# Guivernoir/ICS-WT-PhysicsEngine

Hardware: AMD Instinct MI355X
Metric: reactor-zone-steps/sec (higher is better)
Workload: dtype f64

## Files before the change

ics-wt-physicsengine_amd/csrc/wt_numjac.hpp:

```cpp
#pragma once
#include <hip/hip_runtime.h>
#include <stdint.h>
#include "wt_tables.hpp"
#include "wt_lanes.hpp"
#include "wt_rhs.hpp"
#include "wt_pcr.hpp"

namespace wt {

struct FdCols { double D[3][3]; double S[3][3]; };

struct ZoneProps { double H, iw, phi, kT, rho; bool bpos; };

struct FdBase { double k_lo, k_hi, kd, H_lo, H_hi, C_lo, C_hi, T_lo, T_hi, rho_hi; };

template <bool ROW>
__device__ __forceinline__ FdBase fd_base(const Lane &L, const RK &k, const double y[3], const ZoneProps &b)
{
    FdBase n;
    n.rho_hi = from_hi<ROW, 1>(L, b.rho);
    n.k_hi = k_above(k, b.rho, n.rho_hi);
    n.k_lo = keep_m(L.m_lo[0], from_lo<ROW, 1>(L, n.k_hi));
    n.kd = k_diag(k, n.k_lo, n.k_hi);
    n.H_lo = keep_m(L.m_lo[0], from_lo<ROW, 1>(L, b.H)); n.H_hi = keep_m(L.m_hi[0], from_hi<ROW, 1>(L, b.H));
    n.C_lo = keep_m(L.m_lo[0], from_lo<ROW, 1>(L, y[SCL])); n.C_hi = keep_m(L.m_hi[0], from_hi<ROW, 1>(L, y[SCL]));
    n.T_lo = keep_m(L.m_lo[0], from_lo<ROW, 1>(L, y[STT])); n.T_hi = keep_m(L.m_hi[0], from_hi<ROW, 1>(L, y[STT]));
    return n;
}

template <bool ROW, int SP, class KC>
__device__ __forceinline__ void fd_species_pass(const Lane &L, const KC &kc, const RK &k, const double y[3], const double f[3],
                                                const ZoneProps &b, const FdBase &n, double hcol, bool colmask, bool all_cols,
                                                FdCols &out, bool &bad, double &badval)
{
    const double ypert = y[SP] + hcol;
#pragma unroll
    for (int q = 0; q < 3; ++q)
#pragma unroll
        for (int r = 0; r < 3; ++r) { out.D[q][r] = 0.0; out.S[q][r] = 0.0; }
    auto put = [&](int q, int r, double fn) { out.D[q][r] = fn - f[q]; out.S[q][r] = fmax(fabs(f[q]), fabs(fn)); };
    const double kphi = b.kT * b.phi;
    if constexpr (SP == SPH) {
        PropPH p = prop_pH(kc, k, ypert);
        if (!all_cols && !colmask) { p.H = b.H; p.iw = b.iw; p.phi = b.phi; }
        const double Hx_lo = keep_m(L.m_lo[0], from_lo<ROW, 1>(L, p.H)), Hx_hi = keep_m(L.m_hi[0], from_hi<ROW, 1>(L, p.H));
        put(SPH, 1, row_pH(k, mix3(n.k_lo, n.k_hi, n.kd, n.H_lo, n.H_hi, p.H), p.H, p.iw));
        put(SCL, 1, row_Cl(k, mix3(n.k_lo, n.k_hi, n.kd, n.C_lo, n.C_hi, y[SCL]), y[SCL], b.kT * p.phi));
        put(SPH, 0, row_pH(k, mix3(n.k_lo, n.k_hi, n.kd, Hx_lo, n.H_hi, b.H), b.H, b.iw));
        put(SPH, 2, row_pH(k, mix3(n.k_lo, n.k_hi, n.kd, n.H_lo, Hx_hi, b.H), b.H, b.iw));
    }
    if constexpr (SP == SCL) {
        const double cx = (all_cols || colmask) ? ypert : y[SCL];
        const double Cx_lo = keep_m(L.m_lo[0], from_lo<ROW, 1>(L, cx)), Cx_hi = keep_m(L.m_hi[0], from_hi<ROW, 1>(L, cx));
        put(SCL, 1, row_Cl(k, mix3(n.k_lo, n.k_hi, n.kd, n.C_lo, n.C_hi, cx), cx, kphi));
        put(SCL, 0, row_Cl(k, mix3(n.k_lo, n.k_hi, n.kd, Cx_lo, n.C_hi, y[SCL]), y[SCL], kphi));
        put(SCL, 2, row_Cl(k, mix3(n.k_lo, n.k_hi, n.kd, n.C_lo, Cx_hi, y[SCL]), y[SCL], kphi));
    }
    if constexpr (SP == STT) {
        PropT p = prop_T(kc, ypert);
        if (colmask && p.bad && !bad) { bad = true; badval = ypert; }
        double tx = ypert;
        if (!all_cols && !colmask) { p.kT = b.kT; p.rho = b.rho; tx = y[STT]; }
        const double Tx_lo = keep_m(L.m_lo[0], from_lo<ROW, 1>(L, tx)), Tx_hi = keep_m(L.m_hi[0], from_hi<ROW, 1>(L, tx));
        const double khi_own = k_above(k, p.rho, n.rho_hi);
        const double khi_up = k_above(k, b.rho, from_hi<ROW, 1>(L, p.rho));
        const double klo_own = keep_m(L.m_lo[0], from_lo<ROW, 1>(L, khi_up));
        const double klo_dn = keep_m(L.m_lo[0], from_lo<ROW, 1>(L, khi_own));
        {
            const double kd = k_diag(k, klo_own, khi_own);
            put(SPH, 1, row_pH(k, mix3(klo_own, khi_own, kd, n.H_lo, n.H_hi, b.H), b.H, b.iw));
            put(SCL, 1, row_Cl(k, mix3(klo_own, khi_own, kd, n.C_lo, n.C_hi, y[SCL]), y[SCL], p.kT * b.phi));
            put(STT, 1, row_T(k, mix3(klo_own, khi_own, kd, n.T_lo, n.T_hi, tx), tx));
        }
        {
            const double kd = k_diag(k, klo_dn, n.k_hi);
            put(SPH, 0, row_pH(k, mix3(klo_dn, n.k_hi, kd, n.H_lo, n.H_hi, b.H), b.H, b.iw));
            put(SCL, 0, row_Cl(k, mix3(klo_dn, n.k_hi, kd, n.C_lo, n.C_hi, y[SCL]), y[SCL], kphi));
            put(STT, 0, row_T(k, mix3(klo_dn, n.k_hi, kd, Tx_lo, n.T_hi, y[STT]), y[STT]));
        }
        {
            const double kd = k_diag(k, n.k_lo, khi_up);
            put(SPH, 2, row_pH(k, mix3(n.k_lo, khi_up, kd, n.H_lo, n.H_hi, b.H), b.H, b.iw));
            put(SCL, 2, row_Cl(k, mix3(n.k_lo, khi_up, kd, n.C_lo, n.C_hi, y[SCL]), y[SCL], kphi));
            put(STT, 2, row_T(k, mix3(n.k_lo, khi_up, kd, n.T_lo, Tx_hi, y[STT]), y[STT]));
        }
    }
}

template <bool ROW, int SP>
__device__ __forceinline__ void fd_col_reduce(const Lane &L, const FdCols &c, double &maxd, double &scale)
{
    maxd = -1.0; scale = 0.0;
#pragma unroll
    for (int q = 0; q < 3; ++q) {
        const bool dep_nb = (q == SP) || (SP == STT);
        const bool dep_own = dep_nb || (q == SCL && SP == SPH);
        if (!dep_own) continue;
        double d_lo = 0, s_lo = 0, d_hi = 0, s_hi = 0;
        if (dep_nb) {
            d_lo = from_lo<ROW, 1>(L, c.D[q][2]); s_lo = from_lo<ROW, 1>(L, c.S[q][2]);
            d_hi = from_hi<ROW, 1>(L, c.D[q][0]); s_hi = from_hi<ROW, 1>(L, c.S[q][0]);
        }
        if (dep_nb && L.has_lo && fabs(d_lo) > maxd) { maxd = fabs(d_lo); scale = s_lo; }
        if (fabs(c.D[q][1]) > maxd) { maxd = fabs(c.D[q][1]); scale = c.S[q][1]; }
        if (dep_nb && L.has_hi && fabs(d_hi) > maxd) { maxd = fabs(d_hi); scale = s_hi; }
    }
}

__device__ __forceinline__ double fd_step(double y, double fac, double ysc)
{
    return __dadd_rn(__dadd_rn(y, __dmul_rn(fac, ysc)), -y);
}

template <bool ROW, int SP, class KC>
__device__ __forceinline__ void num_jac_species(const Lane &L, const KC &kc, const RK &k, const double y[3], const double f[3],
                                                const ZoneProps &b, const FdBase &nb, double &fac, FdCols &cols, bool &bad, double &badval)
{
    const double fs = (f[SP] >= 0) ? 1.0 : -1.0;
    const double ysc = fs * fmax(ATOL, fabs(y[SP]));
    double h = fd_step(y[SP], fac, ysc);
    while (WT_RARE(h == 0)) { fac *= 10; h = fd_step(y[SP], fac, ysc); }
    fd_species_pass<ROW, SP>(L, kc, k, y, f, b, nb, h, true, true, cols, bad, badval);
    double maxd, scl;
    fd_col_reduce<ROW, SP>(L, cols, maxd, scl);
    const bool small = maxd < rc::NJ_REJECT * scl;
    if (WT_RARE(__ballot(small) != 0ull)) {
        const double nf = 10 * fac;
        const double hn = fd_step(y[SP], nf, ysc);
        FdCols c2;
        fd_species_pass<ROW, SP>(L, kc, k, y, f, b, nb, hn, small, false, c2, bad, badval);
        double md2, sc2;
        fd_col_reduce<ROW, SP>(L, c2, md2, sc2);
        const bool upd = small && (maxd * sc2 < md2 * scl);
        if (upd) { fac = nf; h = hn; maxd = md2; scl = sc2; }
        const int iu = upd ? 1 : 0;
        const int iu_lo = __shfl_up(iu, 1, 64), iu_hi = __shfl_down(iu, 1, 64);
        const bool upd_lo = L.has_lo && (iu_lo != 0), upd_hi = L.has_hi && (iu_hi != 0);
#pragma unroll
        for (int q = 0; q < 3; ++q) {
            if (upd_lo) cols.D[q][0] = c2.D[q][0];
            if (upd) cols.D[q][1] = c2.D[q][1];
            if (upd_hi) cols.D[q][2] = c2.D[q][2];
        }
    }
    const double h_lo = from_lo<ROW, 1>(L, h), h_hi = from_hi<ROW, 1>(L, h);
    const double ih0 = L.has_lo ? rcp(h_lo) : 0.0, ih1 = rcp(h), ih2 = L.has_hi ? rcp(h_hi) : 0.0;
#pragma unroll
    for (int q = 0; q < 3; ++q) { cols.D[q][0] *= ih0; cols.D[q][1] *= ih1; cols.D[q][2] *= ih2; }
    const bool sm = maxd < rc::NJ_SMALL * scl, bg = maxd > rc::NJ_BIG * scl;
    if (sm) fac *= 10;
    if (bg) fac *= 0.1;
    fac = fmax(fac, rc::NJ_MINF);
}

template <bool ROW, class KTP>
__device__ __forceinline__ void num_jac(const Lane &L, const RKStore &ks, KTP ktab, const double y[3], const double f[3],
                                        double fac[3], bool &have_fac, Jac &J, bool &bad, double &badval, bool &t_dense)
{
    if (!have_fac) { fac[0] = fac[1] = fac[2] = rc::NJ_F0; have_fac = true; }
    FdCols cols;
    ZoneProps b;
    FdBase nb;
    {
        const KT ct = load_kt(ktab());
        const PropT bpt = prop_T(ct, y[STT]);
        b.kT = bpt.kT; b.rho = bpt.rho;
    }
    {
        const KP cp = load_kp(ktab());
        const RK k = fetch_reactor(ks);
        const PropPH bpp = prop_pH(cp, k, y[SPH]);
        b.H = bpp.H; b.iw = bpp.iw; b.phi = bpp.phi; b.bpos = bpp.bpos;
        nb = fd_base<ROW>(L, k, y, b);
        num_jac_species<ROW, SPH>(L, cp, k, y, f, b, nb, fac[SPH], cols, bad, badval);
#pragma unroll
        for (int r = 0; r < 3; ++r) J.pp[r] = cols.D[SPH][r];
        J.cp = cols.D[SCL][1];
    }
    {
        const RK k = fetch_reactor(ks);
        num_jac_species<ROW, SCL>(L, 0, k, y, f, b, nb, fac[SCL], cols, bad, badval);
#pragma unroll
        for (int r = 0; r < 3; ++r) J.cc[r] = cols.D[SCL][r];
    }
    {
        const KT ct = load_kt(ktab());
        const RK k = fetch_reactor(ks);
        num_jac_species<ROW, STT>(L, ct, k, y, f, b, nb, fac[STT], cols, bad, badval);
#pragma unroll
        for (int r = 0; r < 3; ++r) { J.tt[r] = cols.D[STT][r]; J.pt[r] = cols.D[SPH][r]; J.ct[r] = cols.D[SCL][r]; }
        t_dense = jac_t_dense(J) || (ct.dense_bias != 0.0);
    }
}

}
```

ics-wt-physicsengine_amd/csrc/wt_step.hpp:

```cpp
#pragma once
#include <hip/hip_runtime.h>
#include <stdint.h>
#include "wt_tables.hpp"
#include "wt_args.hpp"
#include "wt_lanes.hpp"
#include "wt_rhs.hpp"
#include "wt_pcr.hpp"
#include "wt_numjac.hpp"
#include "wt_queue.hpp"

namespace wt {

template <bool ROW, int LV = 6>
__device__ __forceinline__ double rms3(const Lane &L, const double x[3], const double sc[3])
{
    double s = 0.0;
#pragma unroll
    for (int q = 0; q < 3; ++q) { const double v = x[q] * rcp(sc[q]); s += v * v; }
    return sqrt_k(div_by(seg_sum<ROW, LV>(L, s), L.d3n));
}

__device__ __forceinline__ double ulp_above(double t)
{
    return __longlong_as_double(__double_as_longlong(t) + 1) - t;
}

__device__ __forceinline__ double predict_factor(double h_abs, bool have_old, double h_abs_old,
                                                 double error_norm, double error_norm_old)
{
    double mult = 1.0;
    const double ie = rcp(error_norm);
    if (have_old && error_norm != 0) mult = h_abs * rcp(h_abs_old) * root4(error_norm_old * ie);
    return fmin(1.0, mult) * root4(ie);
}

struct Flag {
    uint32_t &w; const uint32_t m;
    __device__ __forceinline__ operator bool() const { return (w & m) != 0u; }
    __device__ __forceinline__ Flag &operator=(bool v) { w = v ? (w | m) : (w & ~m); return *this; }
    __device__ __forceinline__ Flag &operator=(const Flag &o) { return *this = (bool)o; }
    __device__ __forceinline__ Flag &operator|=(bool v) { w = v ? (w | m) : w; return *this; }
};

enum Phase : int {
    PH_OUTER_BEGIN = 0,
    PH_INIT_STEP,
    PH_F1,
    PH_STEP_BEGIN,
    PH_ATTEMPT,
    PH_NEWTON,
    PH_ERR_REFINE,
    PH_FNEW,
    PH_DONE
};

struct SolverCounters { int nfev, njev, nlu, nsteps, nrej; };

template <int LV> struct LdsMap {
    static constexpr int RK_DOUBLES = RK_UNI * rk_maxr(LV) + rk_lane_doubles(LV);
    static constexpr int HIST_DOUBLES = rk_maxr(LV);
    static constexpr int F_DOUBLES = FSlots<LV>::LDS_SLOTS * 64;
    static constexpr int IO_DOUBLES = (int)((sizeof(wts::StepIO) + 7) / 8);
    static constexpr int TAIL_DOUBLES = F_DOUBLES > IO_DOUBLES ? F_DOUBLES : IO_DOUBLES;
    static constexpr int X_OFF = RK_DOUBLES + HIST_DOUBLES, X_DOUBLES = 64;
    static constexpr int F_OFF = (X_OFF + X_DOUBLES + 1) & ~1;
    static constexpr int TOTAL = F_OFF + TAIL_DOUBLES;
    static_assert(X_OFF >= (LV >= 2 ? (1 << (LV - 2)) : 0), "reads below the exchange row must stay inside the allocation");
};

template <bool ROW, int NS>
__device__ __forceinline__ void rhs_points(const Lane &L, const RKStore &ks, ArgPtr pa, const double (*y)[3], double (*F)[3], bool *bad)
{
    PropPH pp[NS]; PropT pt[NS];
    {
        ArgPtr a = fresh(pa);
        const KP c = load_kp(&a->kt);
        const RK k = fetch_reactor(ks);
        double x[NS];
#pragma unroll
        for (int s = 0; s < NS; ++s) x[s] = y[s][SPH];
        prop_pH_n<NS>(c, k, x, pp);
    }
    __builtin_amdgcn_sched_barrier(0);
    {
        ArgPtr a = fresh(pa);
        const KT c = load_kt(&a->kt);
        double x[NS];
#pragma unroll
        for (int s = 0; s < NS; ++s) x[s] = y[s][STT];
        prop_T_n<NS>(c, x, pt);
#pragma unroll
        for (int s = 0; s < NS; ++s) bad[s] = pt[s].bad;
    }
    {
        const RK k = fetch_reactor(ks);
#pragma unroll
        for (int s = 0; s < NS; ++s)
            rhs_rows<ROW>(L, k, pp[s].H, pp[s].iw, pp[s].bpos, pt[s].kT * pp[s].phi, pt[s].rho, y[s][SCL], y[s][STT], F[s]);
    }
}

__host__ __device__ constexpr bool first_attempt_in_probe_trip(int , bool ) { return true; }

template <int LV, bool ROW>
__device__ __forceinline__ void run_item(ArgPtr pa, const Lane &L, double *lds, int group, int step0, int cnt)
{
    using M = LdsMap<LV>;
    ArgPtr a = fresh(pa);
    const int n_zones = L.n, R = a->R;
    const int lane = threadIdx.x & 63, seg = lane / n_zones;
    const int64_t q_first = (int64_t)group * R;
    const int64_t q_end = a->q_ctrl ? a->N : a->r1;
    const bool present = (seg < R) && (q_first + seg < q_end);
    const int64_t r = present ? (int64_t)a->perm[q_first + seg] : 0;
    const int64_t idx = r * n_zones + L.z;
    const double dt = a->dt;
    const int step_limit = a->step_limit, sens_on = a->sens.on, plc_on = a->sens.plc_on;
    const bool want_diag = a->wave_diag != nullptr;
    const RKStore ks = {lds + seg, lds + RK_UNI * rk_maxr(LV) + lane, rk_maxr(LV), L.m_lo[0], L.m_hi[0], rk_lane_in_lds(LV)};
    int *hist0 = reinterpret_cast<int *>(lds + M::RK_DOUBLES);
    int *rix = hist0 + rk_maxr(LV);
    double *lds_factors = lds + M::F_OFF;
    wts::StepIO &io = *reinterpret_cast<wts::StepIO *>(lds_factors);

    double y0[3] = {7.0, 1.0, 20.0};
    double f[3] = {0, 0, 0};
    double t_out = 0;
    double dH = 0, dR = 0, dK = 0, badval = 0;
    double flow_used = 0;
    uint32_t st = 0;
    bool frozen = !present, f_valid = false, wrote_k = false, raised = false;
    int steps_done = 0, reads_done = 0, cost_acc = 0;
    SolverCounters last_cnt = {0, 0, 0, 0, 0};
    int diag_trips = 0, diag_newton = 0;
#ifdef WT_STAMPS
    int diag_fact = 0, diag_jac = 0, diag_f3 = 0;
#define WT_COUNT(c) ++(c)
#else
    constexpr int diag_fact = 0, diag_jac = 0, diag_f3 = 0;
#define WT_COUNT(c) do { } while (0)
#endif
#ifdef WT_STAMPS
    long long sec[8] = {0, 0, 0, 0, 0, 0, 0, 0}; long long tprev = __builtin_amdgcn_s_memtime();
#define WT_STAMP(i) do { const long long tn_ = __builtin_amdgcn_s_memtime(); sec[i] += tn_ - tprev; tprev = tn_; } while (0)
#else
#define WT_STAMP(i) do { } while (0)
#endif
    const long long clk0 = want_diag ? __builtin_amdgcn_s_memtime() : 0, wall0 = want_diag ? __builtin_amdgcn_s_memrealtime() : 0;
    if (present) {
        st = a->status[r];
        if (st & (ST_T_RANGE | ST_T_RANGE_POST)) frozen = true;
        y0[SPH] = a->pH[idx]; y0[SCL] = a->Cl[idx]; y0[STT] = a->T[idx];
        t_out = a->time[r];
        const double *bc = a->sched ? a->sched + (int64_t)(a->first_step + step0) * NB * a->N : a->bc;
        RK k0; load_reactor(a->par, bc, a->N, r, n_zones, k0); mask_reactor_for_lane(L, k0);
        park_reactor(ks, k0);
        if (sens_on && L.z == 0) hist0[seg] = a->sens.hist_value ? a->sens.hist_pos[r] : 0;
        if (L.z == 0) rix[seg] = (int)r;
    }

    for (int k = 0; k < cnt; ++k) {
        bool stepped = false;
        if (!frozen) {
          if (WT_RARE(seg_any(L, !(isfinite(y0[0]) && isfinite(y0[1]) && isfinite(y0[2]))))) { st |= ST_NONFINITE; frozen = true; }
          else {
            double yc[3], W[3][3];
            double aux[3] = {0, 0, 0};
            constexpr bool HELD = LV <= 5;
            typedef Held<HELD> AReg64;
            AReg64 Qa[3][3], y_old_a[3], sol_t_old_a, sol_h_a;
#pragma unroll
            for (int q = 0; q < 3; ++q) { y_old_a[q].init(); Qa[q][0].init(); Qa[q][1].init(); Qa[q][2].init(); }
            sol_t_old_a.init(); sol_h_a.init();
            Jac J;
            JacA<(LV <= 4)> ja; ja.init();
            FStore<LV> F;
            F.cell = (LdsDouble2 *)lds_factors + lane;
            uint32_t fl = 1u << 4;
            Flag have_fac{fl, 1u << 0}, have_old{fl, 1u << 1}, have_old_l{fl, 1u << 2}, have_sol{fl, 1u << 3}, current_jac{fl, 1u << 4},
                 have_lu{fl, 1u << 5}, rejected{fl, 1u << 6}, keep_h{fl, 1u << 7}, have_norm_old{fl, 1u << 8}, have_rate{fl, 1u << 9},
                 bad{fl, 1u << 10}, failed{fl, 1u << 11}, fv{fl, 1u << 12}, need_jac{fl, 1u << 13},
                 limit_hit{fl, 1u << 16}, pend_f{fl, 1u << 17}, jac_after_fnew{fl, 1u << 18},
                 j_dense{fl, 1u << 19};
            fv = f_valid;
            AReg64 fac_a[3]; fac_a[0].init(); fac_a[1].init(); fac_a[2].init();
            double t = t_out, t_bound = t_out + dt, max_step = fmin(dt, 10.0);
            double h = 0, t_new = 0, h_abs = 0, h_abs_l = 0, min_step = 0;
            AReg64 h_abs_old_a, err_old_a, h_abs_old_l_a, err_old_l_a;
            h_abs_old_a.init(); err_old_a.init(); h_abs_old_l_a.init(); err_old_l_a.init();
            int kk = 0, n_iter = 0; double dW_norm_old = 0, rate = 0;
            double error_norm = 0, safety = 0;
            double d0 = 0, d1 = 0, h0 = 0;
            SolverCounters cnt_s = {0, 0, 0, 0, 0};
            int attempts = 0;
            int badstage = 0;
            int phase = PH_OUTER_BEGIN;
#pragma unroll
            for (int q = 0; q < 3; ++q) { yc[q] = y0[q]; W[0][q] = W[1][q] = W[2][q] = 0.0; }

            auto initial_step_first_half = [&]() {
                double sc[3];
#pragma unroll
                for (int q = 0; q < 3; ++q) sc[q] = ATOL + fabs(yc[q]) * RTOL;
                d0 = rms3<ROW, LV>(L, yc, sc); d1 = rms3<ROW, LV>(L, f, sc);
                h0 = (d0 < 1e-5 || d1 < 1e-5) ? 1e-6 : 0.01 * d0 * rcp(d1);
                h0 = fmin(h0, fabs(t_bound - t));
#pragma unroll
                for (int q = 0; q < 3; ++q) aux[q] = yc[q] + h0 * f[q];
            };
            auto reject_step = [&]() {
                const double fct = predict_factor(h_abs_l, have_old_l, h_abs_old_l_a.get(), error_norm, err_old_l_a.get());
                h_abs_l *= fmax(MIN_FACTOR, safety * fct);
                have_lu = false; rejected = true; cnt_s.nrej++;
                phase = PH_ATTEMPT;
            };
            auto accept_step = [&]() {
                const bool recompute_jac = (n_iter > 2) && have_rate && (rate > 1e-3);
                double fct = predict_factor(h_abs_l, have_old_l, h_abs_old_l_a.get(), error_norm, err_old_l_a.get());
                fct = fmin(MAX_FACTOR, safety * fct);
                if (!recompute_jac && fct < 1.2) fct = 1.0; else have_lu = false;
                h_abs_old_a.set(h_abs);
                err_old_a.set(error_norm);
                have_old = true;
                h_abs = h_abs_l * fct;
                const KZ kz = lit_kz(); const KA ka = lit_ka();
#pragma unroll
                for (int q = 0; q < 3; ++q) {
                    const ZRow z = z_of_w(kz, W, q);
                    y_old_a[q].set(yc[q]);
                    Qa[q][0].set(z.z0 * ka.P[0] + z.z1 * ka.P[3] + z.z2 * ka.P[6]);
                    Qa[q][1].set(z.z0 * ka.P[1] + z.z1 * ka.P[4] + z.z2 * ka.P[7]);
                    Qa[q][2].set(z.z0 * ka.P[2] + z.z1 * ka.P[5] + z.z2 * ka.P[8]);
                    yc[q] = yc[q] + z.z2;
                }
                sol_t_old_a.set(t); sol_h_a.set(t_new - t); have_sol = true;
                t = t_new;
                cnt_s.nsteps++; cnt_s.nfev++;
                pend_f = true; fv = false;
                current_jac = recompute_jac;
                const bool more = (t - t_bound) < 0;
                if (recompute_jac || !more) { jac_after_fnew = recompute_jac; phase = PH_FNEW; }
                else phase = PH_STEP_BEGIN;
            };

            if (fv) {
                cnt_s.nfev++;
                phase = PH_INIT_STEP;
            }

            WT_STAMP(0);
            while (true) {
                if (__ballot(phase != PH_DONE) == 0ull) break;
                if (phase == PH_INIT_STEP) {
                    initial_step_first_half();
                    phase = PH_F1;
                }
                if (phase == PH_STEP_BEGIN) {
                    min_step = 10 * fabs(ulp_above(t));
                    if (h_abs > max_step) { h_abs_l = max_step; have_old_l = false; }
                    else if (h_abs < min_step) { h_abs_l = min_step; have_old_l = false; }
                    else { h_abs_l = h_abs; have_old_l = have_old; h_abs_old_l_a.set(h_abs_old_a.get()); err_old_l_a.set(err_old_a.get()); }
                    rejected = false; keep_h = false;
                    phase = PH_ATTEMPT;
                }
                if (phase == PH_ATTEMPT) {
                    if (!keep_h) {
                        if (WT_RARE(step_limit > 0 && attempts >= step_limit)) { failed = true; limit_hit = true; phase = PH_DONE; }
                        else if (WT_RARE(h_abs_l < min_step)) { failed = true; phase = PH_DONE; }
                        else {
                            attempts++;
                            h = h_abs_l;
                            t_new = t + h;
                            if (t_new - t_bound > 0) t_new = t_bound;
                            h = t_new - t;
                            h_abs_l = fabs(h);
                        }
                    }
                    if (phase == PH_ATTEMPT) {
                        keep_h = false;
                        double Z0[3][3];
                        if (!have_sol) {
#pragma unroll
                            for (int s = 0; s < 3; ++s)
#pragma unroll
                                for (int q = 0; q < 3; ++q) Z0[s][q] = 0.0;
                        } else {
                            const double sol_t_old = sol_t_old_a.get(), isol = rcp(sol_h_a.get());
                            double Q[3][3], y_old[3];
#pragma unroll
                            for (int q = 0; q < 3; ++q) { y_old[q] = y_old_a[q].get(); Q[q][0] = Qa[q][0].get(); Q[q][1] = Qa[q][1].get(); Q[q][2] = Qa[q][2].get(); }
                            const KG kg = load_kg(&fresh(pa)->rt);
                            const double cs[3] = {kg.C0, kg.C1, 1.0};
#pragma unroll
                            for (int s = 0; s < 3; ++s) {
                                const double x = ((t + h * cs[s]) - sol_t_old) * isol;
                                const double p1 = x * x, p2 = p1 * x;
#pragma unroll
                                for (int q = 0; q < 3; ++q)
                                    Z0[s][q] = (__builtin_fma(Q[q][2], p2, __builtin_fma(Q[q][0], x, Q[q][1] * p1)) + y_old[q]) - yc[q];
                            }
                        }
                        const KN kn0 = load_kn(&fresh(pa)->rt);
#pragma unroll
                        for (int q = 0; q < 3; ++q) {
                            W[0][q] = kn0.TI[0] * Z0[0][q] + kn0.TI[1] * Z0[1][q] + kn0.TI[2] * Z0[2][q];
                            W[1][q] = kn0.TI[3] * Z0[0][q] + kn0.TI[4] * Z0[1][q] + kn0.TI[5] * Z0[2][q];
                            W[2][q] = kn0.TI[6] * Z0[0][q] + kn0.TI[7] * Z0[1][q] + kn0.TI[8] * Z0[2][q];
                        }
                        kk = 0; have_norm_old = false; have_rate = false; rate = 0.0;
                        phase = PH_NEWTON;
                    }
                }
                WT_STAMP(1);
                const bool newton = (phase == PH_NEWTON);
                diag_trips++;
                const bool eval0 = (phase == PH_OUTER_BEGIN || phase == PH_F1 || phase == PH_ERR_REFINE || phase == PH_FNEW || newton);
                const bool eval3 = newton && pend_f;
                double ye[3][3], Fe[3][3];
#pragma unroll
                for (int q = 0; q < 3; ++q) {
                    double p0 = yc[q];
                    if (phase == PH_F1) p0 = aux[q];
                    if (phase == PH_ERR_REFINE) p0 = yc[q] + aux[q];
                    ye[0][q] = p0;
                }
                auto stage_points = [&]() {
                    const KZ kzp = load_kz(&fresh(pa)->rt);
#pragma unroll
                    for (int q = 0; q < 3; ++q) {
                        const ZRow z = z_of_w(kzp, W, q);
                        if (newton) ye[0][q] = yc[q] + z.z0;
                        ye[1][q] = yc[q] + z.z1; ye[2][q] = yc[q] + z.z2;
                    }
                };
                if constexpr (LV >= 5) stage_points();
                bool b0 = false, b1 = false, b2 = false, b3 = false;
                if (__ballot(newton) != 0ull) {
                    if constexpr (LV < 5) stage_points();
                    bool bb[3];
                    rhs_points<ROW, 3>(L, ks, pa, ye, Fe, bb);
                    b0 = bb[0] && eval0; b1 = bb[1] && newton; b2 = bb[2] && newton;
                    if (eval0 && phase != PH_FNEW) cnt_s.nfev++;
                    if (newton) cnt_s.nfev += 2;
                } else if (__ballot(eval0) != 0ull) {
                    bool bb[1];
                    rhs_points<ROW, 1>(L, ks, pa, ye, Fe, bb);
                    b0 = bb[0] && eval0;
                    if (eval0 && phase != PH_FNEW) cnt_s.nfev++;
                }
                if (__ballot(eval3) != 0ull) {
                    WT_COUNT(diag_f3);
                    double fy[1][3]; bool bb[1];
                    rhs_points<ROW, 1>(L, ks, pa, &yc, fy, bb);
                    b3 = bb[0] && eval3;
                    if (eval3) {
                        pend_f = false;
#pragma unroll
                        for (int q = 0; q < 3; ++q) f[q] = fy[0][q];
                    }
                }
                if (WT_RARE(__ballot(b0 || b1 || b2 || b3) != 0ull)) {
                    const bool mine = b0 || b1 || b2 || b3;
                    if (mine && !bad) {
                        badstage = b3 ? 0 : (b0 ? 1 : (b1 ? 2 : 3));
                        badval = b3 ? yc[STT] : (b0 ? ye[0][STT] : (b1 ? ye[1][STT] : ye[2][STT]));
                    }
                    bad |= mine;
                    if (seg_any(L, bad)) { raised = true; phase = PH_DONE; }
                }

                if (WT_RARE(phase == PH_OUTER_BEGIN)) {
#pragma unroll
                    for (int q = 0; q < 3; ++q) f[q] = Fe[0][q];
                    phase = PH_INIT_STEP;
                } else if (phase == PH_F1) {
                    double sc[3], df[3];
#pragma unroll
                    for (int q = 0; q < 3; ++q) { sc[q] = ATOL + fabs(yc[q]) * RTOL; df[q] = Fe[0][q] - f[q]; }
                    const double d2 = rms3<ROW, LV>(L, df, sc) * rcp(h0);
                    double h1;
                    if (d1 <= 1e-15 && d2 <= 1e-15) h1 = fmax(1e-6, h0 * 1e-3);
                    else h1 = root4(0.01 * rcp(fmax(d1, d2)));
                    h_abs = fmin(fmin(100 * h0, h1), fmin(fabs(t_bound - t), max_step));
                    need_jac = true;
                    if constexpr (!first_attempt_in_probe_trip(LV, ROW)) phase = PH_STEP_BEGIN;
                    else {
                        min_step = 10 * fabs(ulp_above(t));
                        h_abs_l = (h_abs < min_step) ? min_step : h_abs;
                        attempts++;
                        h = h_abs_l;
                        t_new = t + h;
                        if (t_new - t_bound > 0) t_new = t_bound;
                        h = t_new - t;
                        h_abs_l = fabs(h);
#pragma unroll
                        for (int s = 0; s < 3; ++s)
#pragma unroll
                            for (int q = 0; q < 3; ++q) Fe[s][q] = f[q];
                        cnt_s.nfev += 3;
                        phase = PH_NEWTON;
                    }
                } else if (phase == PH_FNEW) {
#pragma unroll
                    for (int q = 0; q < 3; ++q) f[q] = Fe[0][q];
                    pend_f = false;
                    fv = true;
                    if (jac_after_fnew) { need_jac = true; jac_after_fnew = false; }
                    phase = ((t - t_bound) < 0) ? PH_STEP_BEGIN : PH_DONE;
                }

                WT_STAMP(3);
#ifdef WT_STAMPS
                if (__ballot(need_jac) != 0ull) WT_COUNT(diag_jac);
#endif
                if (need_jac) {
                    bool jbad = false, hf = have_fac, jd = false; double jval = 0;
                    asm volatile("" ::: "memory");
                    double fac[3] = {fac_a[0].get(), fac_a[1].get(), fac_a[2].get()};
                    num_jac<ROW>(L, ks, [&]() { return &fresh(pa)->kt; }, yc, f, fac, hf, J, jbad, jval, jd); cnt_s.njev++;
                    fac_a[0].set(fac[0]); fac_a[1].set(fac[1]); fac_a[2].set(fac[2]);
                    have_fac = hf;
                    j_dense = jd;
                    ja.put(J);
                    need_jac = false;
                    if (WT_RARE(seg_any(L, jbad))) {
                        if (jbad) { badstage = 0; badval = jval; }
                        bad |= jbad; raised = true; phase = PH_DONE;
                    }
                }
                WT_STAMP(5);
#ifdef WT_STAMPS
                if (__ballot(phase == PH_NEWTON && !have_lu) != 0ull) WT_COUNT(diag_fact);
#endif
                if (phase == PH_NEWTON && !have_lu) {
                    { Jac Jb; ja.bands(Jb); factorize<ROW, LV>(L, Jb, h, F); } have_lu = true; cnt_s.nlu += 2;
                }

                WT_STAMP(2);
                if (__ballot(phase == PH_NEWTON) != 0ull) diag_newton++;
                if (phase == PH_NEWTON) {
                    Jac Jc; ja.coupling(Jc);
                    bool finite = true;
#pragma unroll
                    for (int s = 0; s < 3; ++s)
#pragma unroll
                        for (int q = 0; q < 3; ++q) finite = finite && isfinite(Fe[s][q]);
                    bool conv = false, diverged = false;
                    if (WT_RARE(!seg_all(L, finite))) {
                        diverged = true;
                    } else {
                        const double ih = rcp(h);
                        const RTabPtr rt = &fresh(pa)->rt;
                        const KN kn = load_kn(rt); const KZ kz = load_kz(rt);
                        const double M_real = kn.mu_r * ih, Mcr = kn.mu_cr * ih, Mci = kn.mu_ci * ih;
                        double fr[3], fcr[3], fci[3], scale[3];
#pragma unroll
                        for (int q = 0; q < 3; ++q) {
                            scale[q] = kz.atol + fabs(yc[q]) * kz.rtol;
                            fr[q] = (Fe[0][q] * kn.TI[0] + Fe[1][q] * kn.TI[1] + Fe[2][q] * kn.TI[2]) - M_real * W[0][q];
                            const double re = Fe[0][q] * kn.TI[3] + Fe[1][q] * kn.TI[4] + Fe[2][q] * kn.TI[5];
                            const double im = Fe[0][q] * kn.TI[6] + Fe[1][q] * kn.TI[7] + Fe[2][q] * kn.TI[8];
                            fcr[q] = re - (Mcr * W[1][q] - Mci * W[2][q]);
                            fci[q] = im - (Mcr * W[2][q] + Mci * W[1][q]);
                        }
                        solve_rc<ROW, LV>(L, Jc, F, fr, fcr, fci, __ballot(j_dense) == 0ull);
                        double ssum = 0.0;
#pragma unroll
                        for (int q = 0; q < 3; ++q) {
                            const double is = rcp(scale[q]);
                            const double u = fr[q] * is, v = fcr[q] * is, w = fci[q] * is;
                            ssum += u * u + v * v + w * w;
                        }
                        const double dW_norm = sqrt_k(div_by(seg_sum<ROW, LV>(L, ssum), L.d9n));
                        if (have_norm_old) { rate = dW_norm * rcp(dW_norm_old); have_rate = true; }
                        const double i1r = rcp(1 - rate);
                        if (have_rate && (rate >= 1 || powi6(rate, NEWTON_MAXITER - kk) * i1r * dW_norm > kn.newton_tol)) {
                            diverged = true;
                        } else {
#pragma unroll
                            for (int q = 0; q < 3; ++q) { W[0][q] += fr[q]; W[1][q] += fcr[q]; W[2][q] += fci[q]; }
                            if (dW_norm == 0 || (have_rate && rate * i1r * dW_norm < kn.newton_tol)) conv = true;
                            dW_norm_old = dW_norm; have_norm_old = true;
                        }
                    }
                    n_iter = kk + 1;
                    kk++;
                    if (!conv && !diverged && kk == NEWTON_MAXITER) diverged = true;
                    if (WT_RARE(diverged)) {
                        if (current_jac) { h_abs_l *= 0.5; have_lu = false; cnt_s.nrej++; phase = PH_ATTEMPT; }
                        else { need_jac = true; current_jac = true; have_lu = false; keep_h = true; phase = PH_ATTEMPT; }
                    } else if (conv) {
                        double err[3], esc[3];
                        const double ih_e = rcp(h);
                        const KZ kze = lit_kz(); const KE ke = lit_ke();
#pragma unroll
                        for (int q = 0; q < 3; ++q) {
                            const ZRow z = z_of_w(kze, W, q);
                            const double ZE = (z.z0 * ke.E0 + z.z1 * ke.E1 + z.z2 * ke.E2) * ih_e;
                            err[q] = f[q] + ZE;
                            esc[q] = kze.atol + fmax(fabs(yc[q]), fabs(yc[q] + z.z2)) * kze.rtol;
                        }
                        solve_real<ROW, LV>(L, Jc, F, err, __ballot(j_dense) == 0ull);
                        error_norm = rms3<ROW, LV>(L, err, esc);
                        safety = 0.9 * (2 * NEWTON_MAXITER + 1) / (2 * NEWTON_MAXITER + n_iter);
                        if (WT_RARE(rejected && error_norm > 1)) {
#pragma unroll
                            for (int q = 0; q < 3; ++q) aux[q] = err[q];
                            phase = PH_ERR_REFINE;
                        } else if (WT_RARE(error_norm > 1)) {
                            reject_step();
                        } else {
                            accept_step();
                        }
                    }
                } else if (WT_RARE(phase == PH_ERR_REFINE)) {
                    Jac Jc; ja.coupling(Jc);
                    double err[3], esc[3];
                    const double ih_e = rcp(h);
                    const KZ kze = lit_kz(); const KE ke = lit_ke();
#pragma unroll
                    for (int q = 0; q < 3; ++q) {
                        const ZRow z = z_of_w(kze, W, q);
                        const double ZE = (z.z0 * ke.E0 + z.z1 * ke.E1 + z.z2 * ke.E2) * ih_e;
                        err[q] = Fe[0][q] + ZE;
                        esc[q] = kze.atol + fmax(fabs(yc[q]), fabs(yc[q] + z.z2)) * kze.rtol;
                    }
                    solve_real<ROW, LV>(L, Jc, F, err, __ballot(j_dense) == 0ull);
                    error_norm = rms3<ROW, LV>(L, err, esc);
                    if (error_norm > 1) reject_step(); else accept_step();
                }
                WT_STAMP(4);
            }
            last_cnt = cnt_s;
            cost_acc += cnt_s.nfev;

            if (WT_RARE(raised)) {
                st |= ST_T_RANGE; frozen = true;
                double v = badval; int best = 1 << 30;
#pragma unroll 1
                for (int sidx = 0; sidx < 5; ++sidx) {
                    const unsigned long long m = __ballot(bad && badstage == sidx) & L.segmask;
                    if (m != 0ull && best == (1 << 30)) { best = sidx; v = __shfl(badval, (int)__builtin_ctzll(m), 64); }
                }
                badval = v;
                raised = false;
            } else {
                if (failed) st |= ST_SOLVER_FAILED;
                if (limit_hit) st |= ST_STEP_LIMIT;
#pragma unroll
                for (int q = 0; q < 3; ++q) y0[q] = yc[q];
                stepped = true; steps_done++;
                t_out = t_out + dt;
                flow_used = ks.uni[15 * ks.stride];
                double dHv; PropT pt;
                {
                    ArgPtr a2 = fresh(pa);
                    const KP cp = load_kp(&a2->kt); const KT ct = load_kt(&a2->kt);
                    dHv = exp10_k(cp, -y0[SPH]); pt = prop_T(ct, y0[STT]);
                }
                dH = dHv;
                dR = pt.rho;
                bool clamped = false;
                if (WT_RARE(seg_any(L, pt.bad))) {
                    st |= ST_T_RANGE_POST; frozen = true;
                    const unsigned long long m = __ballot(pt.bad) & L.segmask;
                    badval = __shfl(y0[STT], (int)__builtin_ctzll(m), 64);
                } else {
                    dK = pt.kT; wrote_k = true;
                    if (WT_RARE(seg_any(L, y0[SPH] < 0 || y0[SPH] > 14))) { st |= ST_CLAMP_PH; y0[SPH] = fmin(fmax(y0[SPH], 0.0), 14.0); clamped = true; }
                    if (WT_RARE(seg_any(L, y0[SCL] < 0))) { st |= ST_CLAMP_CL; y0[SCL] = fmax(y0[SCL], 0.0); clamped = true; }
                    if (WT_RARE(seg_any(L, y0[STT] < 0 || y0[STT] > 100))) { st |= ST_CLAMP_T; y0[STT] = fmin(fmax(y0[STT], 0.0), 100.0); clamped = true; }
                    f_valid = fv && !clamped && !failed;
                }
            }
          }
        }

        WT_STAMP(6);
        if constexpr (prog_in_item(LV)) {
          if (WT_RARE(fresh(pa)->scr.on)) {
            ArgPtr s = fresh(pa);
            static_assert(M::TAIL_DOUBLES >= wtsc::STAGE_DOUBLES, "the score program stages the zones' state in the factor store");
            const bool live = present && stepped && !(st & ST_T_RANGE_POST);
            wtsc::evaluate(s->scr, live, L.z, n_zones, lane, L.base, r, t_out, y0, lds_factors,
                           s->scr.step0 + s->first_step + step0 + k);
          }
        }
        if constexpr (prog_in_item(LV)) {
          const int dst_on = fresh(pa)->dst.on, trn_on = fresh(pa)->trn.on;
          if (WT_RARE((dst_on | trn_on) != 0)) {
            ArgPtr d = fresh(pa);
            const bool live = present && stepped && !(st & ST_T_RANGE_POST);
            bool reload = false;
            double q0 = 0.0;
            if (trn_on && d->trn.jct.on && present && !L.has_hi) q0 = d->bc[r];
            if (dst_on) {
                if (live && L.z == 0) wtd::evaluate(d->dst, r, t_out, d->bc, d->N, ExpK());
                reload = live;
            }
            static_assert(M::TAIL_DOUBLES >= wtr::PARK_Q * wtr::PARK_SEGS, "a junction program parks the outlets in the factor store");
            if (trn_on) reload = wtr::feed(d->trn, present, live, !L.has_hi, seg, n_zones, r, t_out, y0, q0, d->bc, d->N, lds_factors, JctK()) || reload;
            __syncthreads();
            if (reload) {
                RK k1; load_reactor(d->par, d->bc, d->N, r, n_zones, k1); mask_reactor_for_lane(L, k1);
                park_reactor(ks, k1);
                f_valid = false;
            }
          }
        }
        if (sens_on) {
            ArgPtr b = fresh(pa);
            __syncthreads();
            if (seg < R) {
                const bool live = stepped && !(st & ST_T_RANGE_POST);
                if (L.z == 0) {
                    io.stepped[seg] = live ? 1 : 0;
                    if (live) reads_done++;
                    io.t_after[seg] = t_out;
                    io.tap[0][seg] = (float)y0[SPH]; io.tap[2][seg] = (float)y0[SCL]; io.tap[4][seg] = (float)y0[STT];
                    io.tap[6][seg] = (float)flow_used;
                }
                if (!L.has_hi) { io.tap[1][seg] = (float)y0[SPH]; io.tap[3][seg] = (float)y0[SCL]; io.tap[5][seg] = (float)y0[STT]; }
            }
            __syncthreads();
            if constexpr (prog_in_item(LV)) wts::suite_step(b->sens, b->ins, io, rix, R, hist0, k, wtsv::Program());
            else wts::suite_step(b->sens, b->ins, io, rix, R, hist0, k);
            if (plc_on) {
                const int gs = b->first_step + step0 + k;
                const bool scan = ((gs + 1) % b->sens.scan_every == 0) || (gs + 1 == b->call_steps);
                __syncthreads();
                if constexpr (prog_in_item(LV)) {
                  if (scan && WT_RARE(fresh(pa)->wir.on)) {
                    ArgPtr wp = fresh(pa);
                    wtw::route(wp->wir, wp->trn.length, lane < R && io.stepped[lane], lane, rix, io);
                  }
                }
                if (lane < R && io.stepped[lane]) {
                    const int64_t rr = rix[lane];
                    const double lt = b->sens.pack.loop_time[rr];
                    if (scan) {
                        const bool inj = prog_in_item(LV) && WT_RARE(fresh(pa)->inj.on);
                        if (inj) wti::tamper_sensors(fresh(pa)->inj, rr, &io.val[0][lane], &io.fault[0][lane], wts::RMAX, lt + dt);
                        wtp::pack_inputs(b->sens.pack, rr, &io.val[0][lane], &io.fault[0][lane], wts::RMAX, lt);
                        double c[3];
                        const bool act = prog_in_item(LV) && WT_RARE(fresh(pa)->act.on);
                        const double row0 = act ? b->sens.cmd.bc[rr] : 0.0;
                        double inlet_v;
                        if (inj) inlet_v = wtp::apply_commands(b->sens.cmd, rr, c, wti::command_tamper(fresh(pa)->inj, rr, lt + dt));
                        else inlet_v = wtp::apply_commands(b->sens.cmd, rr, c);
                        if (prog_in_item(LV) && WT_RARE(fresh(pa)->alm.on)) wta::override_commands(fresh(pa)->alm, b->sens.cmd, rr, c);
                        if (act) wtv::actuate(fresh(pa)->act, b->sens.cmd, rr, c, inlet_v, row0, lt + dt);
                        io.cmd[0][lane] = c[0]; io.cmd[1][lane] = c[1]; io.cmd[2][lane] = c[2];
                    }
                    b->sens.pack.loop_time[rr] = lt + dt;
                }
                int owned = 0;
                if constexpr (prog_in_item(LV)) {
                  if (scan && WT_RARE(fresh(pa)->tun.on) && lane < R && io.stepped[lane]) {
                    ArgPtr up = fresh(pa);
                    const int64_t rr = rix[lane];
                    owned = wtu::tune_execute(up->tun, up->ctl, rr, &io.val[0][lane], &io.fault[0][lane], wts::RMAX, up->sens.pack.loop_time[rr]);
                  }
                }
                if (scan && WT_RARE(fresh(pa)->ctl.on) && lane < R && io.stepped[lane]) {
                    ArgPtr cp = fresh(pa);
                    const int64_t rr = rix[lane];
                    wtc::pi_execute(cp->ctl, rr, &io.val[0][lane], &io.fault[0][lane], wts::RMAX, cp->sens.pack.loop_time[rr], owned);
                }
                if (prog_in_item(LV) && scan && WT_RARE(fresh(pa)->alm.on) && lane < R && io.stepped[lane]) {
                    ArgPtr ap = fresh(pa);
                    const int64_t rr = rix[lane];
                    wta::evaluate(ap->alm, rr, ap->sens.N, &io.val[0][lane], &io.fault[0][lane], wts::RMAX, ap->sens.out_value,
                                  ap->sens.out_fault, ap->sens.pack.loop_time[rr]);
                }
                if constexpr (prog_in_item(LV)) {
                  if (scan && WT_RARE(fresh(pa)->det.on) && lane < R && io.stepped[lane]) {
                    ArgPtr dp = fresh(pa);
                    const int64_t rr = rix[lane];
                    wtk::evaluate(dp->det, rr, dp->sens.N, &io.val[0][lane], &io.fault[0][lane], wts::RMAX, dp->sens.out_value,
                                  dp->sens.out_fault, dp->sens.pack.loop_time[rr]);
                  }
                }
                if constexpr (prog_in_item(LV)) {
                  if (scan && WT_RARE(fresh(pa)->trd.on) && lane < R && io.stepped[lane]) {
                    ArgPtr tp = fresh(pa);
                    const int64_t rr = rix[lane];
                    wtt::record(*tp, rr, &io.val[0][lane], &io.fault[0][lane], &io.cmd[0][lane], wts::RMAX, tp->sens.pack.loop_time[rr]);
                  }
                }
                if (scan) {
                    __syncthreads();
                    if (present && io.stepped[seg]) {
                        RK k0; load_reactor(b->par, b->bc, b->N, r, n_zones, k0, &io.cmd[0][seg], wts::RMAX); mask_reactor_for_lane(L, k0);
                        park_reactor(ks, k0);
                        f_valid = false;
                    }
                }
            }
            __syncthreads();
        }
        if constexpr (x_in_item(LV)) {
          if (WT_RARE(fresh(pa)->x_on)) {
            ArgPtr x = fresh(pa);
            const int gs = x->first_step + step0 + k;
            if (x->rec_pH) {
                const unsigned m = (unsigned)x->rec_phase + (unsigned)gs + 1u, every = (unsigned)x->rec_every;
                const unsigned slot = (unsigned)x->rec_slot0 + m / every - 1u;
                if (m % every == 0u && slot < (unsigned)x->rec_cap && present) {
                    const int64_t row = (int64_t)slot * x->N;
                    const int64_t o = row * n_zones + idx;
                    x->rec_pH[o] = y0[SPH]; x->rec_Cl[o] = y0[SCL]; x->rec_T[o] = y0[STT];
                    if (L.z == 0) {
                        x->rec_time[row + r] = t_out;
                        x->rec_flow[row + r] = steps_done > 0 ? flow_used : x->flow[r];
                        x->rec_status[row + r] = st;
                    }
                }
            }
            if (x->sched && k + 1 < cnt) {
                if (present) {
                    RK k1; load_reactor(x->par, x->sched + (int64_t)(gs + 1) * NB * x->N, x->N, r, n_zones, k1);
                    mask_reactor_for_lane(L, k1);
                    park_reactor(ks, k1);
                }
                f_valid = false;
            }
          }
        }
        WT_STAMP(7);
    }

    ArgPtr c = fresh(pa);
    if (present) {
        if (steps_done > 0) {
            c->pH[idx] = y0[SPH]; c->Cl[idx] = y0[SCL]; c->T[idx] = y0[STT];
            c->dH[idx] = dH; c->dRho[idx] = dR;
            if (wrote_k) c->dK[idx] = dK;
        }
        if (L.z == 0) {
            if (steps_done > 0) {
                c->time[r] = t_out;
                c->flow[r] = flow_used;
                if (c->stats) {
                    int32_t *o = c->stats + r * 5;
                    o[0] = last_cnt.nfev; o[1] = last_cnt.njev; o[2] = last_cnt.nlu; o[3] = last_cnt.nsteps; o[4] = last_cnt.nrej;
                }
                if (sens_on && c->sens.hist_value) c->sens.hist_pos[r] = hist0[seg] + reads_done;
            }
            c->status[r] = st;
            if (st & (ST_T_RANGE | ST_T_RANGE_POST)) c->bad_T[r] = badval;
            if (c->cost && cost_acc > 0) c->cost[r] += cost_acc;
        }
    }
    if (want_diag && lane == 0) {
        unsigned long long *o = reinterpret_cast<unsigned long long *>(c->wave_diag + (int64_t)group * WT_DIAG_SLOTS);
        atomicAdd(o + 0, (unsigned long long)diag_trips); atomicAdd(o + 1, (unsigned long long)diag_newton);
        atomicAdd(o + 2, (unsigned long long)(__builtin_amdgcn_s_memtime() - clk0));
        atomicAdd(o + 3, (unsigned long long)(__builtin_amdgcn_s_memrealtime() - wall0));
        atomicAdd(o + 4, (unsigned long long)diag_fact); atomicAdd(o + 5, (unsigned long long)diag_jac);
        atomicAdd(o + 6, (unsigned long long)diag_f3); atomicAdd(o + 7, 1ull);
#ifdef WT_STAMPS
        for (int i = 0; i < 8; ++i) atomicAdd(o + 8 + i, (unsigned long long)sec[i]);
#endif
    }
}

}
```

Before: 1.726 billion.

## Restructure Radau step loop to skip redundant RHS and property evaluations

Several schedule changes go into the implicit solver loop. The outer-begin RHS evaluation is hoisted ahead of the first trip, and its base properties are handed to the numerical Jacobian so they are not recomputed. The pending f evaluation is folded into the Newton stage block as a fourth point. The last accepted step skips the step-size prediction and dense-output bookkeeping and ends directly instead of passing through an FNEW phase. Per-step derived outputs (dH, rho, kT) are computed once per work item rather than every step. Together these aim to cut transcendental property evaluations and warp-divergent extra RHS calls, at the cost of more registers, more complex control flow, and a separate out-of-range temperature check at the final accept.

```diff
diff --git a/ics-wt-physicsengine_amd/csrc/wt_numjac.hpp b/ics-wt-physicsengine_amd/csrc/wt_numjac.hpp
--- a/ics-wt-physicsengine_amd/csrc/wt_numjac.hpp
+++ b/ics-wt-physicsengine_amd/csrc/wt_numjac.hpp
@@ -155,13 +155,15 @@
 
 template <bool ROW, class KTP>
 __device__ __forceinline__ void num_jac(const Lane &L, const RKStore &ks, KTP ktab, const double y[3], const double f[3],
-                                        double fac[3], bool &have_fac, Jac &J, bool &bad, double &badval, bool &t_dense)
+                                        double fac[3], bool &have_fac, Jac &J, bool &bad, double &badval, bool &t_dense,
+                                        const ZoneProps *held = nullptr, bool have_held = false)
 {
     if (!have_fac) { fac[0] = fac[1] = fac[2] = rc::NJ_F0; have_fac = true; }
     FdCols cols;
     ZoneProps b;
     FdBase nb;
-    {
+    const bool all_held = held != nullptr && __ballot(!have_held) == 0ull;
+    if (!all_held) {
         const KT ct = load_kt(ktab());
         const PropT bpt = prop_T(ct, y[STT]);
         b.kT = bpt.kT; b.rho = bpt.rho;
@@ -169,8 +171,11 @@
     {
         const KP cp = load_kp(ktab());
         const RK k = fetch_reactor(ks);
-        const PropPH bpp = prop_pH(cp, k, y[SPH]);
-        b.H = bpp.H; b.iw = bpp.iw; b.phi = bpp.phi; b.bpos = bpp.bpos;
+        if (!all_held) {
+            const PropPH bpp = prop_pH(cp, k, y[SPH]);
+            b.H = bpp.H; b.iw = bpp.iw; b.phi = bpp.phi; b.bpos = bpp.bpos;
+        }
+        if (held != nullptr && (all_held || have_held)) b = *held;
         nb = fd_base<ROW>(L, k, y, b);
         num_jac_species<ROW, SPH>(L, cp, k, y, f, b, nb, fac[SPH], cols, bad, badval);
 #pragma unroll
diff --git a/ics-wt-physicsengine_amd/csrc/wt_step.hpp b/ics-wt-physicsengine_amd/csrc/wt_step.hpp
--- a/ics-wt-physicsengine_amd/csrc/wt_step.hpp
+++ b/ics-wt-physicsengine_amd/csrc/wt_step.hpp
@@ -69,7 +69,8 @@
 };
 
 template <bool ROW, int NS>
-__device__ __forceinline__ void rhs_points(const Lane &L, const RKStore &ks, ArgPtr pa, const double (*y)[3], double (*F)[3], bool *bad)
+__device__ __forceinline__ void rhs_points(const Lane &L, const RKStore &ks, ArgPtr pa, const double (*y)[3], double (*F)[3], bool *bad,
+                                           ZoneProps *keep = nullptr)
 {
     PropPH pp[NS]; PropT pt[NS];
     {
@@ -98,9 +99,17 @@
         for (int s = 0; s < NS; ++s)
             rhs_rows<ROW>(L, k, pp[s].H, pp[s].iw, pp[s].bpos, pt[s].kT * pp[s].phi, pt[s].rho, y[s][SCL], y[s][STT], F[s]);
     }
+    if (keep) { keep->H = pp[0].H; keep->iw = pp[0].iw; keep->phi = pp[0].phi; keep->bpos = pp[0].bpos; keep->kT = pt[0].kT; keep->rho = pt[0].rho; }
 }
 
 __host__ __device__ constexpr bool first_attempt_in_probe_trip(int , bool ) { return true; }
+
+__host__ __device__ constexpr bool outer_step_ends_at_accept(int , bool ) { return true; }
+__host__ __device__ constexpr bool outer_begin_ahead_of_first_trip(int , bool ) { return true; }
+__host__ __device__ constexpr bool pending_f_in_stage_block(int , bool ) { return true; }
+__host__ __device__ constexpr bool derived_once_per_item(int , bool ) { return true; }
+__host__ __device__ constexpr bool base_properties_handed_to_num_jac(int LV, bool ) { return LV <= 5; }
+__host__ __device__ constexpr bool lean_last_accept(int , bool ) { return true; }
 
 template <int LV, bool ROW>
 __device__ __forceinline__ void run_item(ArgPtr pa, const Lane &L, double *lds, int group, int step0, int cnt)
@@ -130,6 +139,10 @@
     double flow_used = 0;
     uint32_t st = 0;
     bool frozen = !present, f_valid = false, wrote_k = false, raised = false;
+    bool derive_due = false;
+    constexpr bool END_AT_ACCEPT = outer_step_ends_at_accept(LV, ROW), BEGIN_AHEAD = outer_begin_ahead_of_first_trip(LV, ROW),
+                   PEND_IN_BLOCK = pending_f_in_stage_block(LV, ROW), DERIVE_ONCE = derived_once_per_item(LV, ROW),
+                   HAND_BASE = BEGIN_AHEAD && base_properties_handed_to_num_jac(LV, ROW), LEAN_LAST_ACCEPT = lean_last_accept(LV, ROW);
     int steps_done = 0, reads_done = 0, cost_acc = 0;
     SolverCounters last_cnt = {0, 0, 0, 0, 0};
     int diag_trips = 0, diag_newton = 0;
@@ -181,9 +194,12 @@
                  have_lu{fl, 1u << 5}, rejected{fl, 1u << 6}, keep_h{fl, 1u << 7}, have_norm_old{fl, 1u << 8}, have_rate{fl, 1u << 9},
                  bad{fl, 1u << 10}, failed{fl, 1u << 11}, fv{fl, 1u << 12}, need_jac{fl, 1u << 13},
                  limit_hit{fl, 1u << 16}, pend_f{fl, 1u << 17}, jac_after_fnew{fl, 1u << 18},
-                 j_dense{fl, 1u << 19};
+                 j_dense{fl, 1u << 19},
+                 base_held{fl, 1u << 20}, base_bpos{fl, 1u << 21};
             fv = f_valid;
             AReg64 fac_a[3]; fac_a[0].init(); fac_a[1].init(); fac_a[2].init();
+            AReg64 zb_a[5];
+            if constexpr (HAND_BASE) { zb_a[0].init(); zb_a[1].init(); zb_a[2].init(); zb_a[3].init(); zb_a[4].init(); }
             double t = t_out, t_bound = t_out + dt, max_step = fmin(dt, 10.0);
             double h = 0, t_new = 0, h_abs = 0, h_abs_l = 0, min_step = 0;
             AReg64 h_abs_old_a, err_old_a, h_abs_old_l_a, err_old_l_a;
@@ -216,36 +232,73 @@
             };
             auto accept_step = [&]() {
                 const bool recompute_jac = (n_iter > 2) && have_rate && (rate > 1e-3);
-                double fct = predict_factor(h_abs_l, have_old_l, h_abs_old_l_a.get(), error_norm, err_old_l_a.get());
-                fct = fmin(MAX_FACTOR, safety * fct);
-                if (!recompute_jac && fct < 1.2) fct = 1.0; else have_lu = false;
-                h_abs_old_a.set(h_abs);
-                err_old_a.set(error_norm);
-                have_old = true;
-                h_abs = h_abs_l * fct;
-                const KZ kz = lit_kz(); const KA ka = lit_ka();
-#pragma unroll
-                for (int q = 0; q < 3; ++q) {
-                    const ZRow z = z_of_w(kz, W, q);
-                    y_old_a[q].set(yc[q]);
-                    Qa[q][0].set(z.z0 * ka.P[0] + z.z1 * ka.P[3] + z.z2 * ka.P[6]);
-                    Qa[q][1].set(z.z0 * ka.P[1] + z.z1 * ka.P[4] + z.z2 * ka.P[7]);
-                    Qa[q][2].set(z.z0 * ka.P[2] + z.z1 * ka.P[5] + z.z2 * ka.P[8]);
-                    yc[q] = yc[q] + z.z2;
-                }
-                sol_t_old_a.set(t); sol_h_a.set(t_new - t); have_sol = true;
+                const bool more = (t_new - t_bound) < 0;
+                if (!LEAN_LAST_ACCEPT || more) {
+                    double fct = predict_factor(h_abs_l, have_old_l, h_abs_old_l_a.get(), error_norm, err_old_l_a.get());
+                    fct = fmin(MAX_FACTOR, safety * fct);
+                    if (!recompute_jac && fct < 1.2) fct = 1.0; else have_lu = false;
+                    h_abs_old_a.set(h_abs);
+                    err_old_a.set(error_norm);
+                    have_old = true;
+                    h_abs = h_abs_l * fct;
+                    const KZ kz = lit_kz(); const KA ka = lit_ka();
+#pragma unroll
+                    for (int q = 0; q < 3; ++q) {
+                        const ZRow z = z_of_w(kz, W, q);
+                        y_old_a[q].set(yc[q]);
+                        Qa[q][0].set(z.z0 * ka.P[0] + z.z1 * ka.P[3] + z.z2 * ka.P[6]);
+                        Qa[q][1].set(z.z0 * ka.P[1] + z.z1 * ka.P[4] + z.z2 * ka.P[7]);
+                        Qa[q][2].set(z.z0 * ka.P[2] + z.z1 * ka.P[5] + z.z2 * ka.P[8]);
+                    }
+                    sol_t_old_a.set(t); sol_h_a.set(t_new - t); have_sol = true;
+                }
+                {
+                    const KZ kz = lit_kz();
+#pragma unroll
+                    for (int q = 0; q < 3; ++q) yc[q] = yc[q] + z_of_w(kz, W, q).z2;
+                }
                 t = t_new;
                 cnt_s.nsteps++; cnt_s.nfev++;
                 pend_f = true; fv = false;
                 current_jac = recompute_jac;
-                const bool more = (t - t_bound) < 0;
-                if (recompute_jac || !more) { jac_after_fnew = recompute_jac; phase = PH_FNEW; }
+                if (recompute_jac || (!END_AT_ACCEPT && !more)) { jac_after_fnew = recompute_jac; phase = PH_FNEW; }
+                else if (!more) {
+                    const bool out = (yc[STT] < 0.0) || (yc[STT] > 100.0);
+                    if (WT_RARE(seg_any(L, out))) {
+                        if (out) { badstage = 0; badval = yc[STT]; }
+                        bad |= out; raised = true;
+                    }
+                    phase = PH_DONE;
+                }
                 else phase = PH_STEP_BEGIN;
             };
 
             if (fv) {
                 cnt_s.nfev++;
                 phase = PH_INIT_STEP;
+            }
+            if constexpr (BEGIN_AHEAD) {
+                if (__ballot(phase == PH_OUTER_BEGIN) != 0ull) {
+                    double fy[1][3]; bool bb[1];
+                    ZoneProps zb;
+                    rhs_points<ROW, 1>(L, ks, pa, &yc, fy, bb, HAND_BASE ? &zb : nullptr);
+                    const bool mine = bb[0] && phase == PH_OUTER_BEGIN;
+                    if (phase == PH_OUTER_BEGIN) {
+                        if constexpr (HAND_BASE) {
+                            zb_a[0].set(zb.H); zb_a[1].set(zb.iw); zb_a[2].set(zb.phi); zb_a[3].set(zb.kT); zb_a[4].set(zb.rho);
+                            base_bpos = zb.bpos; base_held = true;
+                        }
+                        cnt_s.nfev++;
+#pragma unroll
+                        for (int q = 0; q < 3; ++q) f[q] = fy[0][q];
+                        phase = PH_INIT_STEP;
+                    }
+                    if (WT_RARE(__ballot(mine) != 0ull)) {
+                        if (mine) { badstage = 1; badval = yc[STT]; }
+                        bad |= mine;
+                        if (seg_any(L, bad)) { raised = true; phase = PH_DONE; }
+                    }
+                }
             }
 
             WT_STAMP(0);
@@ -314,9 +367,10 @@
                 WT_STAMP(1);
                 const bool newton = (phase == PH_NEWTON);
                 diag_trips++;
-                const bool eval0 = (phase == PH_OUTER_BEGIN || phase == PH_F1 || phase == PH_ERR_REFINE || phase == PH_FNEW || newton);
+                const bool eval0 = ((!BEGIN_AHEAD && phase == PH_OUTER_BEGIN) || phase == PH_F1 || phase == PH_ERR_REFINE || phase == PH_FNEW || newton);
                 const bool eval3 = newton && pend_f;
-                double ye[3][3], Fe[3][3];
+                constexpr int NPT = PEND_IN_BLOCK ? 4 : 3;
+                double ye[NPT][3], Fe[NPT][3];
 #pragma unroll
                 for (int q = 0; q < 3; ++q) {
                     double p0 = yc[q];
@@ -337,8 +391,25 @@
                 bool b0 = false, b1 = false, b2 = false, b3 = false;
                 if (__ballot(newton) != 0ull) {
                     if constexpr (LV < 5) stage_points();
-                    bool bb[3];
-                    rhs_points<ROW, 3>(L, ks, pa, ye, Fe, bb);
+                    bool bb[NPT];
+                    bool four = false;
+                    if constexpr (PEND_IN_BLOCK) four = __ballot(eval3) != 0ull;
+                    if (four) {
+                        if constexpr (PEND_IN_BLOCK) {
+                            WT_COUNT(diag_f3);
+#pragma unroll
+                            for (int q = 0; q < 3; ++q) ye[NPT - 1][q] = yc[q];
+                            rhs_points<ROW, NPT>(L, ks, pa, ye, Fe, bb);
+                            b3 = bb[NPT - 1] && eval3;
+                            if (eval3) {
+                                pend_f = false;
+#pragma unroll
+                                for (int q = 0; q < 3; ++q) f[q] = Fe[NPT - 1][q];
+                            }
+                        }
+                    } else {
+                        rhs_points<ROW, 3>(L, ks, pa, ye, Fe, bb);
+                    }
                     b0 = bb[0] && eval0; b1 = bb[1] && newton; b2 = bb[2] && newton;
                     if (eval0 && phase != PH_FNEW) cnt_s.nfev++;
                     if (newton) cnt_s.nfev += 2;
@@ -348,7 +419,7 @@
                     b0 = bb[0] && eval0;
                     if (eval0 && phase != PH_FNEW) cnt_s.nfev++;
                 }
-                if (__ballot(eval3) != 0ull) {
+                if (!PEND_IN_BLOCK && __ballot(eval3) != 0ull) {
                     WT_COUNT(diag_f3);
                     double fy[1][3]; bool bb[1];
                     rhs_points<ROW, 1>(L, ks, pa, &yc, fy, bb);
@@ -369,7 +440,7 @@
                     if (seg_any(L, bad)) { raised = true; phase = PH_DONE; }
                 }
 
-                if (WT_RARE(phase == PH_OUTER_BEGIN)) {
+                if (!BEGIN_AHEAD && WT_RARE(phase == PH_OUTER_BEGIN)) {
 #pragma unroll
                     for (int q = 0; q < 3; ++q) f[q] = Fe[0][q];
                     phase = PH_INIT_STEP;
@@ -417,7 +488,14 @@
                     bool jbad = false, hf = have_fac, jd = false; double jval = 0;
                     asm volatile("" ::: "memory");
                     double fac[3] = {fac_a[0].get(), fac_a[1].get(), fac_a[2].get()};
-                    num_jac<ROW>(L, ks, [&]() { return &fresh(pa)->kt; }, yc, f, fac, hf, J, jbad, jval, jd); cnt_s.njev++;
+                    if constexpr (HAND_BASE) {
+                        const ZoneProps zb = {zb_a[0].get(), zb_a[1].get(), zb_a[2].get(), zb_a[3].get(), zb_a[4].get(), (bool)base_bpos};
+                        num_jac<ROW>(L, ks, [&]() { return &fresh(pa)->kt; }, yc, f, fac, hf, J, jbad, jval, jd, &zb, (bool)base_held);
+                        base_held = false;
+                    } else {
+                        num_jac<ROW>(L, ks, [&]() { return &fresh(pa)->kt; }, yc, f, fac, hf, J, jbad, jval, jd);
+                    }
+                    cnt_s.njev++;
                     fac_a[0].set(fac[0]); fac_a[1].set(fac[1]); fac_a[2].set(fac[2]);
                     have_fac = hf;
                     j_dense = jd;
@@ -547,30 +625,46 @@
             } else {
                 if (failed) st |= ST_SOLVER_FAILED;
                 if (limit_hit) st |= ST_STEP_LIMIT;
+                const double T_before = y0[STT];
 #pragma unroll
                 for (int q = 0; q < 3; ++q) y0[q] = yc[q];
                 stepped = true; steps_done++;
                 t_out = t_out + dt;
                 flow_used = ks.uni[15 * ks.stride];
-                double dHv; PropT pt;
-                {
-                    ArgPtr a2 = fresh(pa);
-                    const KP cp = load_kp(&a2->kt); const KT ct = load_kt(&a2->kt);
-                    dHv = exp10_k(cp, -y0[SPH]); pt = prop_T(ct, y0[STT]);
-                }
-                dH = dHv;
-                dR = pt.rho;
-                bool clamped = false;
-                if (WT_RARE(seg_any(L, pt.bad))) {
-                    st |= ST_T_RANGE_POST; frozen = true;
-                    const unsigned long long m = __ballot(pt.bad) & L.segmask;
-                    badval = __shfl(y0[STT], (int)__builtin_ctzll(m), 64);
+                bool ordinary = false;
+                if constexpr (DERIVE_ONCE) {
+                    const bool odd = (y0[STT] < 0.0) || (y0[STT] > 100.0)
+                                  || (y0[SPH] < 0) || (y0[SPH] > 14) || (y0[SCL] < 0);
+                    ordinary = !WT_RARE(seg_any(L, odd));
+                }
+                if (ordinary) {
+                    derive_due = true;
+                    f_valid = fv && !failed;
                 } else {
-                    dK = pt.kT; wrote_k = true;
-                    if (WT_RARE(seg_any(L, y0[SPH] < 0 || y0[SPH] > 14))) { st |= ST_CLAMP_PH; y0[SPH] = fmin(fmax(y0[SPH], 0.0), 14.0); clamped = true; }
-                    if (WT_RARE(seg_any(L, y0[SCL] < 0))) { st |= ST_CLAMP_CL; y0[SCL] = fmax(y0[SCL], 0.0); clamped = true; }
-                    if (WT_RARE(seg_any(L, y0[STT] < 0 || y0[STT] > 100))) { st |= ST_CLAMP_T; y0[STT] = fmin(fmax(y0[STT], 0.0), 100.0); clamped = true; }
-                    f_valid = fv && !clamped && !failed;
+                    double dHv; PropT pt;
+                    if (DERIVE_ONCE && derive_due) {
+                        dK = prop_T(load_kt(&fresh(pa)->kt), T_before).kT; wrote_k = true;
+                        derive_due = false;
+                    }
+                    {
+                        ArgPtr a2 = fresh(pa);
+                        const KP cp = load_kp(&a2->kt); const KT ct = load_kt(&a2->kt);
+                        dHv = exp10_k(cp, -y0[SPH]); pt = prop_T(ct, y0[STT]);
+                    }
+                    dH = dHv;
+                    dR = pt.rho;
+                    bool clamped = false;
+                    if (WT_RARE(seg_any(L, pt.bad))) {
+                        st |= ST_T_RANGE_POST; frozen = true;
+                        const unsigned long long m = __ballot(pt.bad) & L.segmask;
+                        badval = __shfl(y0[STT], (int)__builtin_ctzll(m), 64);
+                    } else {
+                        dK = pt.kT; wrote_k = true;
+                        if (WT_RARE(seg_any(L, y0[SPH] < 0 || y0[SPH] > 14))) { st |= ST_CLAMP_PH; y0[SPH] = fmin(fmax(y0[SPH], 0.0), 14.0); clamped = true; }
+                        if (WT_RARE(seg_any(L, y0[SCL] < 0))) { st |= ST_CLAMP_CL; y0[SCL] = fmax(y0[SCL], 0.0); clamped = true; }
+                        if (WT_RARE(seg_any(L, y0[STT] < 0 || y0[STT] > 100))) { st |= ST_CLAMP_T; y0[STT] = fmin(fmax(y0[STT], 0.0), 100.0); clamped = true; }
+                        f_valid = fv && !clamped && !failed;
+                    }
                 }
             }
           }
@@ -730,6 +824,14 @@
         WT_STAMP(7);
     }
 
+    if constexpr (DERIVE_ONCE) {
+        if (derive_due) {
+            ArgPtr a2 = fresh(pa);
+            const KP cp = load_kp(&a2->kt); const KT ct = load_kt(&a2->kt);
+            const PropT pt = prop_T(ct, y0[STT]);
+            dH = exp10_k(cp, -y0[SPH]); dR = pt.rho; dK = pt.kT; wrote_k = true;
+        }
+    }
     ArgPtr c = fresh(pa);
     if (present) {
         if (steps_done > 0) {
```

New measurement: 1.777 billion, median of 6. 1.03x the previous value.
